# Hiroki-Maeda/ninwavelets

Hardware: AMD Instinct MI355X
Metric: CWT throughput (epochs*chans*samples*freqs)/s (higher is better)
Workload: dtype f32; 1 GPU; C4 Morse CWT, 512 epochs x 64 ch x 16384 samples x 256 freqs per GPU (4096 epochs at 8 GPUs), complex64 out; wavelet=morse, epochs=512, chans=64, samples=16384, freqs=256, output=cwt, engine=fused, chunk_signals=512, parallelism=dp1 (signals sharded, no collective)

## Files before the change

ninwavelets_amd/csrc/nw_fft_dev.h:

```cpp
#pragma once

#include <type_traits>

#include "nw_dcheck.h"
#include "nw_dft_reg.h"
#include "nw_internal.h"
#include "nw_shape.h"

#ifndef NW_PACK_MAX
#define NW_PACK_MAX 2
#endif
constexpr int kPackMax = NW_PACK_MAX;
constexpr int kPruneMin = 4;
constexpr int kXdmaMinE = 32;
constexpr int kWregMaxE = 16;

namespace nw {
namespace {


__device__ __forceinline__ C2<f2> pk(C2<float> a, C2<float> b) { return {f2{a.re, b.re}, f2{a.im, b.im}}; }
__device__ __forceinline__ C2<float> lo(C2<f2> p) { return {p.re.x, p.im.x}; }
__device__ __forceinline__ C2<float> hi(C2<f2> p) { return {p.re.y, p.im.y}; }

__device__ __forceinline__ double mul_nocontract(double a, double b) {
#pragma clang fp contract(off)
    return a * b;
}
__device__ __forceinline__ double add_nocontract(double a, double b) {
#pragma clang fp contract(off)
    return a + b;
}

template <typename P>
__device__ __forceinline__ P* at(P* base, uint32_t lane_off, uint32_t c = 0) {
    asm volatile("" : "+v"(lane_off));
    return reinterpret_cast<P*>(reinterpret_cast<char*>(base) + (lane_off + c));
}
template <typename P>
__device__ __forceinline__ const P* at(const P* base, uint32_t lane_off, uint32_t c = 0) {
    asm volatile("" : "+v"(lane_off));
    return reinterpret_cast<const P*>(reinterpret_cast<const char*>(base) + (lane_off + c));
}

template <typename T, int R, int N, int NSR, bool SPLIT = false>
__device__ __forceinline__ void twiddle_bases(C2<T>* p, int m, const C2<T>* __restrict__ tw,
                                              const C2<T>* split = nullptr) {
    asm volatile("" : "+v"(m));
#pragma unroll
    for (int k = 0; k < ilog2<R>(); ++k) {
        if constexpr (SPLIT) {
            const uint32_t i = ((uint32_t)m << k) * (uint32_t)(N / NSR);
            p[k] = cmul(split[i >> 5], split[N / 64 + (i & 31)]);
        } else if constexpr (sizeof(T) == 4) {
            const float rev = (float)(m << k) * (1.0f / (float)NSR);
            p[k] = C2<T>{__builtin_amdgcn_cosf(rev), __builtin_amdgcn_sinf(rev)};
        } else {
            p[k] = *at(tw, (uint32_t)m * (uint32_t)((N / NSR) * sizeof(C2<T>)) << k);
        }
    }
}
template <typename T, int R, typename P>
__device__ __forceinline__ void twiddle_dft(C2<T>* v, const C2<P>* p) {
    idft_br_tw<T, R>(v, TwPowers<P, R>(p));
}
template <typename S, int R, int NS, bool FENCE> struct TwTable {
    using scalar = S;
    const C2<S>* tab;
    __device__ __forceinline__ C2<S> lo(int r) const { return tab[(r - 1) * NS]; }
    __device__ __forceinline__ C2<S> hi(int r) const {
        const C2<S> w = tab[(r + R / 2 - 1) * NS];
        if (FENCE && r % 4 == 3) __builtin_amdgcn_sched_barrier(0);
        return w;
    }
};

template <int E> constexpr int kPadG = E < 32 ? 32 : E;
template <int E> __device__ __forceinline__ int lds_idx(int i) { return i + 2 * (i / kPadG<E>); }
template <int E> constexpr int lds_off(int c) { return c + 2 * (c / kPadG<E>); }
template <int N, int E> constexpr int lds_elems() { return N + 2 * (N / kPadG<E>); }

template <int N, int E> struct Geometry {
    static constexpr int T = N / E;
    static constexpr int radix(int p) {
        int done = E;
        for (int i = 1; i < p; ++i) done *= (N / done >= E ? E : N / done);
        const int left = N / done;
        return p == 0 ? E : (left >= E ? E : left);
    }
    static constexpr int npass() {
        int done = E, p = 1;
        while (done < N) {
            done *= (N / done >= E ? E : N / done);
            ++p;
        }
        return p;
    }
    static constexpr int ns(int p) {
        int done = 1;
        for (int i = 0; i < p; ++i) done *= radix(i);
        return done;
    }
};

template <int PG> __device__ __forceinline__ int lds_idx_p(int i) { return i + 2 * (i / PG); }
template <int PG> constexpr int lds_off_p(int c) { return c + 2 * (c / PG); }
template <typename T> constexpr bool kIsPair = !std::is_same<T, Sc<T>>::value;
#ifndef NW_PAIR_PAD16
#define NW_PAIR_PAD16 1
#endif
template <typename T, int N, int E>
constexpr bool kPad16 = NW_PAIR_PAD16 && kIsPair<T> && E == 16 && N / E == 256 && Geometry<N, E>::npass() > 2;
template <typename T, int N, int E, int P> constexpr int kPadX = (kPad16<T, N, E> && P == 1) ? 16 : kPadG<E>;
template <typename T, int N, int E> constexpr int kImgElems = kPad16<T, N, E> ? N + 2 * (N / 16) : lds_elems<N, E>();

template <int OUT, typename T> struct OutT { using type = T; };
template <typename T> struct OutT<NW_OUT_CWT, T> { using type = C2<T>; };
constexpr int kOutXHalf = 1000;
constexpr int kOutPSum = 1001;
constexpr int kOutPhSum = 1002;
constexpr int kOutXSum = 1003;
constexpr int kOutPlvSum = 1004;
template <int OUT> constexpr int kPairAcc = OUT == kOutXSum ? 4 : OUT == kOutPlvSum ? 2 : 1;
struct alignas(16) XHalfSlot { double a, b; };
template <typename T> struct OutT<kOutXHalf, T> { using type = XHalfSlot; };
template <int OUT, typename T>
__device__ __forceinline__ typename OutT<OUT, T>::type out_value(C2<T> y) {
    if constexpr (OUT == NW_OUT_CWT) return y;
    else if constexpr (OUT == NW_OUT_POWER) return y.re * y.re + y.im * y.im;
    else return (T)sqrt(y.re * y.re + y.im * y.im);
}

constexpr int kStoreGlobal = 0, kStoreGlobalNt = 1, kStoreBuffer = 2;
#ifdef NW_LINT_HAZARD_SOFFSET
constexpr bool kSoffsetInField = true;
#else
constexpr bool kSoffsetInField = false;
#endif
template <int SP, typename V>
__device__ __forceinline__ void store_row(V val, void* row, uint32_t lane_off, uint32_t c_off) {
    if constexpr (SP == kStoreBuffer) {
        const __amdgpu_buffer_rsrc_t rs = __builtin_amdgcn_make_buffer_rsrc(
            reinterpret_cast<char*>(row) + (kSoffsetInField ? 0 : c_off), 0, 0x7fffffff, 0x00020000);
        const int so = kSoffsetInField ? (int)c_off : 0;
        if constexpr (sizeof(V) == 16)
            __builtin_amdgcn_raw_buffer_store_b128(__builtin_bit_cast(__attribute__((ext_vector_type(4))) unsigned, val),
                                                   rs, (int)lane_off, so, 2);
        else if constexpr (sizeof(V) == 8)
            __builtin_amdgcn_raw_buffer_store_b64(__builtin_bit_cast(__attribute__((ext_vector_type(2))) unsigned, val),
                                                  rs, (int)lane_off, so, 2);
        else
            __builtin_amdgcn_raw_buffer_store_b32(__builtin_bit_cast(unsigned, val), rs, (int)lane_off, so, 2);
    } else {
        __builtin_nontemporal_store(val, reinterpret_cast<V*>(at(reinterpret_cast<char*>(row), lane_off, c_off)));
    }
}
template <typename O> using StoreVec =
    typename std::conditional<sizeof(O) == 16, float __attribute__((ext_vector_type(4))),
    typename std::conditional<sizeof(O) == 8, float __attribute__((ext_vector_type(2))), float>::type>::type;

template <int OUT, typename T, int SP>
__device__ __forceinline__ void store_pair(void* orow, uint32_t lane_idx, uint32_t c_idx, C2<T> y0, C2<T> y1) {
    using O = typename OutT<OUT, T>::type;
    struct alignas(2 * sizeof(O)) P2 { O a, b; };
#ifdef NW_ABL_NOSTORE
    asm volatile("" ::"v"(y0.re), "v"(y0.im), "v"(y1.re), "v"(y1.im), "v"(lane_idx));
    return;
#endif
    using V = typename std::conditional<sizeof(P2) == 16, float __attribute__((ext_vector_type(4))),
              typename std::conditional<sizeof(P2) == 8, float __attribute__((ext_vector_type(2))),
                                        double __attribute__((ext_vector_type(4)))>::type>::type;
    const P2 pv{out_value<OUT, T>(y0), out_value<OUT, T>(y1)};
    store_row<SP>(__builtin_bit_cast(V, pv), orow, lane_idx * (uint32_t)sizeof(O), c_idx * (uint32_t)sizeof(O));
}
template <int OUT, typename T, int SP>
__device__ __forceinline__ void store_one(void* orow, uint32_t lane_idx, uint32_t c_idx, C2<T> y) {
    using O = typename OutT<OUT, T>::type;
#ifdef NW_ABL_NOSTORE
    asm volatile("" ::"v"(y.re), "v"(y.im), "v"(lane_idx));
    return;
#endif
    if constexpr (SP == kStoreGlobal)
        *at(reinterpret_cast<O*>(orow), lane_idx * (uint32_t)sizeof(O), c_idx * (uint32_t)sizeof(O)) =
            out_value<OUT, T>(y);
    else
        store_row<SP>(__builtin_bit_cast(StoreVec<O>, out_value<OUT, T>(y)), orow, lane_idx * (uint32_t)sizeof(O),
                      c_idx * (uint32_t)sizeof(O));
}

#ifdef NW_STAMPS
constexpr int kStamps = 8;
__device__ unsigned long long g_nw_stamps[kStamps + 1];
struct Stamps {
    unsigned long long last, acc[kStamps];
};
__device__ __forceinline__ unsigned long long nw_now() {
    unsigned long long t;
    __builtin_amdgcn_sched_barrier(0);
    asm volatile("s_memtime %0\n\ts_waitcnt lgkmcnt(0)" : "=s"(t)::"memory");
    __builtin_amdgcn_sched_barrier(0);
    return t;
}
#define NW_STAMP(st, k)                                 \
    do {                                                \
        if (st) {    \
            const unsigned long long now_ = nw_now();   \
            (st)->acc[k] += now_ - (st)->last;          \
            (st)->last = now_;                          \
        }                                               \
    } while (0)
constexpr int kStampsStore = kStamps - 1;
#else
struct Stamps {};
#define NW_STAMP(st, k) ((void)(st))
#endif

template <typename T> struct alignas(2 * sizeof(T)) Pair {
    T a, b;
};

template <int COMP, typename T> __device__ __forceinline__ T& comp(C2<T>& c) {
    if constexpr (COMP == 0) return c.re; else return c.im;
}

template <int N, int E, int P, int OSZ = 8, bool PK = false, bool LN = false> struct PassInfo;
typedef __attribute__((address_space(3))) void lds_void_t;

#ifdef NW_LANE_IMAGE_TU
constexpr bool kLaneImageTU = true;
#else
constexpr bool kLaneImageTU = false;
#endif
template <typename T, int N, int E, int OUT>
constexpr bool kLaneImage = kLaneImageTU && kLaneImageShape<T, N, E> && OUT != kOutXHalf;

template <int OFF0, int STEP, bool WAIT>
__device__ __forceinline__ void addtid_store16(uint32_t m0, const float* d) {
    static_assert(OFF0 >= 0 && OFF0 + 15 * STEP < 65536, "16-bit offset field");
    asm volatile(
        "s_mov_b32 m0, %16\n\ts_nop 0\n\t"
        "ds_write_addtid_b32 %0 offset:%17+0*%18\n\t"
        "ds_write_addtid_b32 %1 offset:%17+1*%18\n\t"
        "ds_write_addtid_b32 %2 offset:%17+2*%18\n\t"
        "ds_write_addtid_b32 %3 offset:%17+3*%18\n\t"
        "ds_write_addtid_b32 %4 offset:%17+4*%18\n\t"
        "ds_write_addtid_b32 %5 offset:%17+5*%18\n\t"
        "ds_write_addtid_b32 %6 offset:%17+6*%18\n\t"
        "ds_write_addtid_b32 %7 offset:%17+7*%18\n\t"
        "ds_write_addtid_b32 %8 offset:%17+8*%18\n\t"
        "ds_write_addtid_b32 %9 offset:%17+9*%18\n\t"
        "ds_write_addtid_b32 %10 offset:%17+10*%18\n\t"
        "ds_write_addtid_b32 %11 offset:%17+11*%18\n\t"
        "ds_write_addtid_b32 %12 offset:%17+12*%18\n\t"
        "ds_write_addtid_b32 %13 offset:%17+13*%18\n\t"
        "ds_write_addtid_b32 %14 offset:%17+14*%18\n\t"
        "ds_write_addtid_b32 %15 offset:%17+15*%18"
        :: "v"(d[0]), "v"(d[1]), "v"(d[2]), "v"(d[3]), "v"(d[4]), "v"(d[5]), "v"(d[6]), "v"(d[7]),
           "v"(d[8]), "v"(d[9]), "v"(d[10]), "v"(d[11]), "v"(d[12]), "v"(d[13]), "v"(d[14]), "v"(d[15]),
           "s"(m0), "i"(OFF0), "i"(STEP)
        : "memory", "m0");
    if constexpr (WAIT) asm volatile("s_waitcnt lgkmcnt(0)" ::: "memory");
}

template <typename T, int N, int E, int P, int COMP>
__device__ __forceinline__ void lane_write(C2<T>* v, T* lds, int t) {
    namespace L = lane_image;
    static_assert(kLaneImageShape<T, N, E> && (P == 0 || P == 1), "the fp32 n = 16384 exchanges");
    static_assert(Geometry<N, E>::T % 64 == 0 && Geometry<N, E>::T == L::kT && L::kRebias == 16,
                  "whole waves (EXEC all ones), 16 stores per M0");
    static_assert(L::kElems <= kImgElems<T, N, E>, "the padded images' region holds these");
    NW_DCHECK_H(__builtin_amdgcn_read_exec() == ~0ull);
    const uint32_t img = (uint32_t)(uintptr_t)(lds_void_t*)lds;
    const int wave = __builtin_amdgcn_readfirstlane(t >> 6);
    float d[E];
#pragma unroll
    for (int k = 0; k < E; ++k) d[k] = comp<COMP>(v[bitrev<E>(k)]);
    if constexpr (P == 0) {
        addtid_store16<L::off_01(0), L::off_01(1) - L::off_01(0), false>(img + L::m0_01(wave), d);
        addtid_store16<L::off_01(16), L::off_01(1) - L::off_01(0), true>(img + L::m0_01(wave), d + 16);
    } else {
        static_assert(PassInfo<N, E, P, 16>::R == E && PassInfo<N, E, P, 16>::Q == 1, "one radix-E butterfly per thread");
        addtid_store16<L::off_12(0), L::off_12(1) - L::off_12(0), false>(img + L::m0_12(wave, 0), d);
        addtid_store16<L::off_12(16), L::off_12(17) - L::off_12(16), true>(img + L::m0_12(wave, 16), d + 16);
    }
}

template <typename T, int N, int E, int P, int COMP, bool LN = false>
__device__ __forceinline__ void lds_write(C2<T>* v, T* lds, int t) {
    using G = Geometry<N, E>;
    constexpr int PG = kPadX<T, N, E, P + 1>;
    if constexpr (LN) {
        lane_write<T, N, E, P, COMP>(v, lds, t);
    } else if constexpr (P == 0) {
        NW_DCHECK_H(lds_idx_p<PG>(t * E + E - 1) < kImgElems<T, N, E>);
        Pair<T>* dst = reinterpret_cast<Pair<T>*>(lds + lds_idx_p<PG>(t * E));
#pragma unroll
        for (int u = 0; u < E / 2; ++u)
            dst[u] = Pair<T>{comp<COMP>(v[bitrev<E>(2 * u)]), comp<COMP>(v[bitrev<E>(2 * u + 1)])};
    } else {
        constexpr int R = G::radix(P);
        constexpr int NS = G::ns(P);
        constexpr int Q = E / R;
#pragma unroll
        for (int q = 0; q < Q; ++q) {
            const int j = PassInfo<N, E, P, 16, kIsPair<T>>::bfly(t, q);
            NW_DCHECK_H(lds_idx_p<PG>((j / NS) * NS * R + j % NS) + lds_off_p<PG>((R - 1) * NS) < kImgElems<T, N, E>);
            T* dst = lds + lds_idx_p<PG>((j / NS) * NS * R + j % NS);
#pragma unroll
            for (int i = 0; i < R; ++i) dst[lds_off_p<PG>(bitrev<R>(i) * NS)] = comp<COMP>(v[q * R + i]);
        }
    }
}

template <int N, int E, int P, int OSZ, bool PK, bool LN> struct PassInfo {
    using G = Geometry<N, E>;
    static constexpr int R = G::radix(P);
    static constexpr int NS = G::ns(P);
    static constexpr int Q = E / R;
    static constexpr int STRIDE = N / R;
    static constexpr bool LAST = (P == G::npass() - 1);
    static constexpr bool PAIRED = LAST && Q == 2 && OSZ <= 8;
    static_assert(STRIDE % E == 0 && NS % E == 0, "pad must stay linear");
    static constexpr bool SWZ = PAIRED && G::T == 512 && kPadG<E> == 32 && !LN;
    static constexpr bool REMAP = PK && NW_PAIR_PAD16 && P == 1 && !LAST && E == 16 && G::T == 256 && Q == 1;
    __device__ static __forceinline__ int bfly(int t, int q) {
        if constexpr (SWZ) return 2 * (((t >> 5) << 4) + (((t >> 4) & 1) << 8) + (t & 15)) + q;
        if constexpr (REMAP) return ((t >> 5) << 4) + (((t >> 4) & 1) << 7) + (t & 15);
        return PAIRED ? Q * t + q : t + q * G::T;
    }
};

template <typename T, int N, int E> struct Tab1 {
    using I = PassInfo<N, E, 1>;
    using S = Sc<T>;
    static constexpr int NS = I::NS, R = I::R;
    static constexpr int COUNT = Geometry<N, E>::npass() >= 2 ? NS * (R - 1) : 0;
#ifdef NW_TAB1_F64_16384
    static constexpr bool BIG = sizeof(S) == 8 && N == 16384 && E == 32;
#else
    static constexpr bool BIG = false;
#endif
    static constexpr bool ON = COUNT > 0 && (COUNT * (int)sizeof(C2<S>) <= 8192 || BIG);
    static constexpr int BYTES = ON ? COUNT * (int)sizeof(C2<S>) : 0;
    static_assert((kImgElems<T, N, E> * sizeof(T)) % 16 == 0, "table alignment");
    __device__ static __forceinline__ const C2<S>* table(const T* lds) {
        return reinterpret_cast<const C2<S>*>(lds + kImgElems<T, N, E>);
    }
    __device__ static __forceinline__ void fill(T* lds, const C2<S>* __restrict__ tw, int t) {
        if constexpr (ON) {
            C2<S>* tab = reinterpret_cast<C2<S>*>(lds + kImgElems<T, N, E>);
            for (int i = t; i < COUNT; i += Geometry<N, E>::T) {
                const int jj = i % NS, r = i / NS + 1;
                tab[i] = tw[(jj * r * (N / (NS * R))) % N];
            }
        }
    }
};

template <typename T, int N, int E, int P, int COMP, int OSZ, bool LN = false>
__device__ __forceinline__ void lds_read(C2<T>* v, const T* lds, int t) {
    using I = PassInfo<N, E, P, OSZ, kIsPair<T>, LN>;
    constexpr int R = I::R, Q = I::Q;
    constexpr int PG = kPadX<T, N, E, P>;
    if constexpr (LN) {
        namespace L = lane_image;
        if constexpr (P == 1) {
            static_assert(Q == 1 && R == E && !I::PAIRED, "pass 1: butterfly t, slots t + 512 r");
            const T* src = lds + L::rbase_01(I::bfly(t, 0));
#pragma unroll
            for (int r = 0; r < R; ++r) comp<COMP>(v[r]) = src[L::roff_01(r)];
        } else {
            static_assert(P == 2 && Q == 2 && I::PAIRED && I::STRIDE == 1024, "pass 2: pairs 2t, 2t + 1, slots j2 + 1024 r");
            const T* src = lds + L::rbase_12(I::bfly(t, 0));
#pragma unroll
            for (int r = 0; r < R; ++r) {
                const Pair<T> pr = *reinterpret_cast<const Pair<T>*>(src + L::roff_12(r));
                comp<COMP>(v[r]) = pr.a;
                comp<COMP>(v[R + r]) = pr.b;
            }
        }
    } else if constexpr (I::PAIRED) {
        NW_DCHECK_H(lds_idx_p<PG>(I::bfly(t, 0)) + (Q - 1) + lds_off_p<PG>((R - 1) * I::STRIDE) < kImgElems<T, N, E>);
        const T* src = lds + lds_idx_p<PG>(I::bfly(t, 0));
#pragma unroll
        for (int q = 0; q < Q; q += 2)
#pragma unroll
            for (int r = 0; r < R; ++r) {
                const Pair<T> pr = *reinterpret_cast<const Pair<T>*>(src + q + lds_off_p<PG>(r * I::STRIDE));
                comp<COMP>(v[q * R + r]) = pr.a;
                comp<COMP>(v[(q + 1) * R + r]) = pr.b;
            }
    } else {
#pragma unroll
        for (int q = 0; q < Q; ++q) {
            NW_DCHECK_H(lds_idx_p<PG>(I::bfly(t, q)) + lds_off_p<PG>((R - 1) * I::STRIDE) < kImgElems<T, N, E>);
            const T* src = lds + lds_idx_p<PG>(I::bfly(t, q));
#pragma unroll
            for (int r = 0; r < R; ++r) comp<COMP>(v[q * R + r]) = src[lds_off_p<PG>(r * I::STRIDE)];
        }
    }
}

__device__ __forceinline__ void lds_barrier() {
    __builtin_amdgcn_s_waitcnt(0xC07F);
    __builtin_amdgcn_s_barrier();
}

typedef __attribute__((address_space(1))) void gbl_void_t;

template <typename T, int N, int TT>
__device__ __forceinline__ void dma_x(const C2<T>* xs, void* dst, int t, int nround = 1 << 30) {
    constexpr int CH = (N / 2) * (int)sizeof(C2<T>) / 16;
    static_assert(CH % TT == 0, "whole DMA rounds");
    const int wave_base = __builtin_amdgcn_readfirstlane((t & ~63) * 16);
    const uint32_t lane_off = (uint32_t)t * 16u;
#pragma unroll
    for (int i = 0; i < CH / TT; ++i) {
        if (i >= nround) break;
        const char* chunk = reinterpret_cast<const char*>(xs) + (size_t)i * TT * 16;
        asm volatile("" : "+s"(chunk));
        const uint32_t lds_addr = (uint32_t)(uintptr_t)(lds_void_t*)(reinterpret_cast<char*>(dst) + i * TT * 16 + wave_base);
        asm volatile("s_mov_b32 m0, %0\n\ts_nop 0\n\tglobal_load_lds_dwordx4 %1, %2"
                     :: "s"(lds_addr), "v"(lane_off), "s"(chunk) : "memory", "m0");
    }
}

__device__ __forceinline__ unsigned long long sload_u64(const void* p) {
    unsigned long long u;
    asm volatile("s_load_dwordx2 %0, %1, 0x0\n\ts_waitcnt lgkmcnt(0)" : "=s"(u) : "s"(p) : "memory");
    return u;
}
__device__ __forceinline__ C2<float> c2_of_u64(unsigned long long u) {
    return C2<float>{__uint_as_float((unsigned)u), __uint_as_float((unsigned)(u >> 32))};
}
template <typename T> __device__ __forceinline__ C2<T> sload_c2(const C2<T>* p) {
    if constexpr (sizeof(T) == 4) {
        unsigned long long u;
        asm volatile("s_load_dwordx2 %0, %1, 0x0\n\ts_waitcnt lgkmcnt(0)" : "=s"(u) : "s"(p) : "memory");
        return C2<T>{__uint_as_float((unsigned)u), __uint_as_float((unsigned)(u >> 32))};
    } else {
        typedef unsigned long long u2 __attribute__((ext_vector_type(2)));
        u2 u;
        asm volatile("s_load_dwordx4 %0, %1, 0x0\n\ts_waitcnt lgkmcnt(0)" : "=s"(u) : "s"(p) : "memory");
        return C2<T>{__longlong_as_double((long long)u.x), __longlong_as_double((long long)u.y)};
    }
}

template <int V>
__device__ __forceinline__ void wait_vmcnt() {
    static_assert(V >= 0 && V < 64, "vmcnt range");
    __builtin_amdgcn_s_waitcnt((V & 0xF) | ((V >> 4) << 14) | 0x70 | 0xF00);
}

template <int CTRL> __device__ __forceinline__ float dpp_f(float v) {
    return __int_as_float(__builtin_amdgcn_mov_dpp(__float_as_int(v), CTRL, 0xF, 0xF, false));
}
template <int CTRL> __device__ __forceinline__ double dpp_f(double v) {
    const long long b = __double_as_longlong(v);
    const int lo = __builtin_amdgcn_mov_dpp((int)(b & 0xffffffffLL), CTRL, 0xF, 0xF, false);
    const int hi = __builtin_amdgcn_mov_dpp((int)(b >> 32), CTRL, 0xF, 0xF, false);
    return __longlong_as_double(((long long)hi << 32) | (unsigned int)lo);
}
template <int D, typename F> __device__ __forceinline__ void xpose2(F& a, F& b, bool hi) {
    constexpr int CTRL = D == 1 ? 0xB1 : 0x4E;
    const F recv = dpp_f<CTRL>(hi ? a : b);
    if (hi) a = recv; else b = recv;
}
template <typename F> __device__ __forceinline__ void xpose2(C2<F>& a, C2<F>& b, bool hi, int d) {
    if (d == 1) { xpose2<1>(a.re, b.re, hi); xpose2<1>(a.im, b.im, hi); }
    else { xpose2<2>(a.re, b.re, hi); xpose2<2>(a.im, b.im, hi); }
}

template <typename T, int N, int E, int OUT, int SP = kStoreGlobal>
struct LastStores {
    using O = typename OutT<OUT, T>::type;
    using I = PassInfo<N, E, Geometry<N, E>::npass() - 1, (int)sizeof(O), false, kLaneImage<T, N, E, OUT>>;
    static constexpr int R = I::R, Q = I::Q;
    static constexpr int STEP = I::PAIRED ? 2 : 1;
    static constexpr int PACK_W = (int)(16 / sizeof(O));
    static constexpr int PACK = (!I::PAIRED && PACK_W <= kPackMax && R % PACK_W == 0) ? PACK_W : 1;
    static_assert(PACK == 1 || PACK == 2 || PACK == 4, "pack");
    static constexpr int COUNT = PACK > 1 ? Q * R / PACK : Q / STEP * R;
    __device__ static __forceinline__ void all(const C2<T>* v, void* orow, int t) {
        if constexpr (PACK == 1) {
            chunk<0, 1>(v, orow, t);
        } else {
            const int c = t & (PACK - 1);
            const uint32_t lane = (uint32_t)((t & ~(PACK - 1)) + I::NS * c) * (uint32_t)sizeof(O);
#pragma unroll
            for (int qg = 0; qg < Q * (R / PACK); ++qg) {
                const int q = qg / (R / PACK), g = qg % (R / PACK);
                O val[PACK];
#pragma unroll
                for (int b = 0; b < PACK; ++b) val[b] = out_value<OUT, T>(v[q * R + bitrev<R>(g * PACK + b)]);
                if constexpr (PACK >= 2) {
                    const bool hi1 = c & 1;
#pragma unroll
                    for (int b = 0; b < PACK; b += 2) xpose_any<1>(val[b], val[b + 1], hi1);
                }
                if constexpr (PACK == 4) {
                    const bool hi2 = c & 2;
                    xpose_any<2>(val[0], val[2], hi2);
                    xpose_any<2>(val[1], val[3], hi2);
                }
                using V = float __attribute__((ext_vector_type(4)));
                struct alignas(16) P16 { O a[PACK]; };
                P16 pk;
#pragma unroll
                for (int b = 0; b < PACK; ++b) pk.a[b] = val[b];
#ifdef NW_ABL_NOSTORE
                asm volatile("" ::"v"(__builtin_bit_cast(V, pk)));
#else
                store_row<SP>(__builtin_bit_cast(V, pk), orow, lane,
                              (uint32_t)((q * Geometry<N, E>::T + g * PACK * I::NS) * sizeof(O)));
#endif
            }
        }
    }
    template <int D, typename F> __device__ static __forceinline__ void xpose_any(F& a, F& b, bool hi) {
        if constexpr (std::is_same<F, float>::value || std::is_same<F, double>::value) xpose2<D>(a, b, hi);
        else xpose2(a, b, hi, D);
    }
    template <int K>
    __device__ static __forceinline__ void one(const C2<T>* o, void* orow, int t) {
        constexpr int q = (K / R) * STEP, i = K % R;
        const uint32_t lane = (uint32_t)I::bfly(t, 0);
        constexpr uint32_t c = (uint32_t)((I::PAIRED ? q : q * Geometry<N, E>::T) + bitrev<R>(i) * I::NS);
        NW_DCHECK_H(lane + c + (I::PAIRED ? 1u : 0u) < (uint32_t)N);
        if constexpr (I::PAIRED)
            store_pair<OUT, T, SP>(orow, lane, c, o[q * R + i], o[(q + 1) * R + i]);
        else
            store_one<OUT, T, SP>(orow, lane, c, o[q * R + i]);
    }
    template <int C, int NCH, int K = C * COUNT / NCH>
    __device__ static __forceinline__ void chunk(const C2<T>* o, void* orow, int t) {
        if constexpr (K < (C + 1) * COUNT / NCH) {
            one<K>(o, orow, t);
            chunk<C, NCH, K + 1>(o, orow, t);
        }
    }
};



template <typename T, int E, bool REALW>
constexpr bool kXDMA = E >= (sizeof(T) == 4 ? kXdmaMinE : 32) && REALW;
template <typename T> __device__ __forceinline__ int dma_rounds_for(int nz) {
    return (nz * (int)sizeof(C2<T>) + 15) / 16;
}

template <typename T, int N, int E> struct TwSplit {
    static constexpr bool ON = std::is_same<T, double>::value && N >= 2048 && N <= 4096;
    static constexpr int NHI = N / 64, COUNT = NHI + 32;
    static constexpr int OFFSET = kImgElems<T, N, E> * (int)sizeof(T) + Tab1<T, N, E>::BYTES;
    static_assert(OFFSET % 16 == 0, "table alignment");
    static constexpr int BYTES = ON ? COUNT * (int)sizeof(C2<T>) : 0;
    __device__ static __forceinline__ const C2<T>* table(const T* lds) {
        return reinterpret_cast<const C2<T>*>(reinterpret_cast<const char*>(lds) + OFFSET);
    }
    __device__ static __forceinline__ void fill(T* lds, const C2<T>* __restrict__ tw, int t) {
        if constexpr (ON) {
            C2<T>* tab = reinterpret_cast<C2<T>*>(reinterpret_cast<char*>(lds) + OFFSET);
            for (int i = t; i < COUNT; i += Geometry<N, E>::T) tab[i] = i < NHI ? tw[i * 32] : tw[i - NHI];
        }
    }
};
template <typename T, int N, int E> constexpr int kLdsBytes =
    kImgElems<T, N, E> * (int)sizeof(T) + Tab1<T, N, E>::BYTES + TwSplit<T, N, E>::BYTES;


template <typename T, int N, int E, int OUT, int P, bool XD, int SP = kStoreGlobal>
__device__ __forceinline__ void passes_from(C2<T>* v, T* lds, int t, const C2<Sc<T>>* __restrict__ tw, C2<T>* x,
                                            const C2<T>* xs_next, void* ocur,
                                            Stamps* st, void* ocur2 = nullptr, int dma_rounds = 1 << 30,
                                            double* acc = nullptr, const void* xs_next2 = nullptr) {
    using S = Sc<T>;
    constexpr bool PAIRSIG = !std::is_same<T, S>::value;
    constexpr int OSZ = (int)sizeof(typename OutT<OUT, S>::type);
    constexpr bool LN = kLaneImage<T, N, E, OUT>;
    using I = PassInfo<N, E, P, OSZ, kIsPair<T>, LN>;
    if constexpr (P < Geometry<N, E>::npass()) {
        constexpr int R = I::R, Q = I::Q, LR = ilog2<R>();
        constexpr bool TABLED = P == 1 && Tab1<T, N, E>::ON;
        constexpr bool SPLIT = TwSplit<T, N, E>::ON;
        const C2<S>* split = nullptr;
        if constexpr (SPLIT) split = reinterpret_cast<const C2<S>*>(TwSplit<T, N, E>::table(lds));
        C2<S> pb[Q][LR > 0 ? LR : 1];
#ifndef NW_ABL_NOTWIDDLE
        if constexpr (!TABLED && I::PAIRED && Q == 2) {
            twiddle_bases<S, R, N, I::NS * R, SPLIT>(pb[0], I::bfly(t, 0) % I::NS, tw, split);
#pragma unroll
            for (int k = 0; k < LR; ++k) pb[1][k] = cmul(pb[0][k], tw[(N / (I::NS * R)) << k]);
        } else if constexpr (!TABLED) {
#pragma unroll
            for (int q = 0; q < Q; ++q) twiddle_bases<S, R, N, I::NS * R, SPLIT>(pb[q], I::bfly(t, q) % I::NS, tw, split);
        }
#endif
#ifndef NW_ABL_NOEXCH
        lds_barrier();
        lds_write<T, N, E, P - 1, 0, LN>(v, lds, t);
        lds_barrier();
        lds_read<T, N, E, P, 0, OSZ, LN>(v, lds, t);
        lds_barrier();
        lds_write<T, N, E, P - 1, 1, LN>(v, lds, t);
        lds_barrier();
        lds_read<T, N, E, P, 1, OSZ, LN>(v, lds, t);
#else
#pragma unroll
        for (int i = 0; i < E; ++i) asm volatile("" : "+v"(v[i].re), "+v"(v[i].im));
#endif
        if constexpr (I::LAST && XD) {
            if (xs_next) {
                lds_barrier();
                if constexpr (PAIRSIG) {
                    dma_x<S, N, Geometry<N, E>::T>(reinterpret_cast<const C2<S>*>(xs_next), lds, t, dma_rounds);
                    dma_x<S, N, Geometry<N, E>::T>(reinterpret_cast<const C2<S>*>(xs_next2),
                                                   reinterpret_cast<char*>(lds) + (N / 2) * sizeof(C2<S>), t, dma_rounds);
                } else {
                    dma_x<T, N, Geometry<N, E>::T>(xs_next, lds, t, dma_rounds);
                }
                __builtin_amdgcn_sched_barrier(0);
            }
        }
        NW_STAMP(st, 2 * P - 1);
#pragma unroll
        for (int q = 0; q < Q; ++q) {
#ifdef NW_ABL_NOTWIDDLE
            constexpr bool TWIDDLED = false;
#else
            constexpr bool TWIDDLED = true;
#endif
            if constexpr (std::is_same<T, float>::value && Q % 2 == 0 && !(TWIDDLED && TABLED)) {
                if (q % 2 == 0) {
                    C2<f2> pv[R];
#pragma unroll
                    for (int i = 0; i < R; ++i)
                        pv[i] = pk(reinterpret_cast<C2<float>*>(v)[q * R + i],
                                   reinterpret_cast<C2<float>*>(v)[(q + 1) * R + i]);
                    if constexpr (TWIDDLED) {
                        C2<f2> pp[LR > 0 ? LR : 1];
#pragma unroll
                        for (int k = 0; k < LR; ++k)
                            pp[k] = pk(reinterpret_cast<C2<float>*>(pb[q])[k], reinterpret_cast<C2<float>*>(pb[q + 1])[k]);
                        twiddle_dft<f2, R>(pv, pp);
                    } else {
                        idft_br<f2, R>(pv);
                    }
#pragma unroll
                    for (int i = 0; i < R; ++i) {
                        reinterpret_cast<C2<float>*>(v)[q * R + i] = lo(pv[i]);
                        reinterpret_cast<C2<float>*>(v)[(q + 1) * R + i] = hi(pv[i]);
                    }
                }
            } else if constexpr (TWIDDLED && TABLED) {
                idft_br_tw<T, R>(v + q * R, TwTable<S, R, I::NS, true>{Tab1<T, N, E>::table(lds) + I::bfly(t, q) % I::NS});
            } else if constexpr (TWIDDLED) {
                twiddle_dft<T, R>(v + q * R, pb[q]);
            } else {
                idft_br<T, R>(v + q * R);
            }
        }
        NW_STAMP(st, 2 * P);
        if constexpr (I::LAST && OUT == kOutPSum) {
            if constexpr (PAIRSIG) {
#pragma unroll
                for (int e = 0; e < Q * R; ++e) {
                    const C2<S> a{v[e].re.x, v[e].im.x};
                    acc[e] += (double)(a.re * a.re + a.im * a.im);
                }
                if (ocur2) {
#pragma unroll
                    for (int e = 0; e < Q * R; ++e) {
                        const C2<S> b{v[e].re.y, v[e].im.y};
                        acc[e] += (double)(b.re * b.re + b.im * b.im);
                    }
                }
            } else {
#pragma unroll
                for (int e = 0; e < Q * R; ++e) acc[e] += (double)(v[e].re * v[e].re + v[e].im * v[e].im);
            }
        } else if constexpr (I::LAST && OUT == kOutPhSum) {
            static_assert(!PAIRSIG, "partial sums run the single-signal kernel");
#pragma unroll
            for (int e = 0; e < Q * R; ++e) {
                const double re = (double)v[e].re, im = (double)v[e].im;
                if constexpr (sizeof(S) == 8) {
                    const double inv = 1.0 / hypot(re, im);
                    acc[2 * e] += mul_nocontract(re, inv);
                    acc[2 * e + 1] += mul_nocontract(im, inv);
                } else {
                    const double inv = rsqrt(re * re + im * im);
                    acc[2 * e] += mul_nocontract(re, inv);
                    acc[2 * e + 1] += mul_nocontract(im, inv);
                }
            }
        } else if constexpr (I::LAST && (OUT == kOutXSum || OUT == kOutPlvSum)) {
            static_assert(PAIRSIG, "cross-channel partials run the signal-pair kernel");
            NW_DCHECK_H(ocur2 != nullptr);
#pragma unroll
            for (int e = 0; e < Q * R; ++e) {
                double ar = (double)v[e].re.x, ai = (double)v[e].im.x;
                double br = (double)v[e].re.y, bi = (double)v[e].im.y;
                if constexpr (OUT == kOutPlvSum) {
                    const double ia = rsqrt(add_nocontract(mul_nocontract(ar, ar), mul_nocontract(ai, ai)));
                    const double ib = rsqrt(add_nocontract(mul_nocontract(br, br), mul_nocontract(bi, bi)));
                    ar = mul_nocontract(ar, ia), ai = mul_nocontract(ai, ia);
                    br = mul_nocontract(br, ib), bi = mul_nocontract(bi, ib);
                }
                constexpr int NA = kPairAcc<OUT>;
                acc[NA * e] += add_nocontract(mul_nocontract(ar, br), mul_nocontract(ai, bi));
                acc[NA * e + 1] += add_nocontract(mul_nocontract(ai, br), -mul_nocontract(ar, bi));
                if constexpr (OUT == kOutXSum) {
                    acc[NA * e + 2] += add_nocontract(mul_nocontract(ar, ar), mul_nocontract(ai, ai));
                    acc[NA * e + 3] += add_nocontract(mul_nocontract(br, br), mul_nocontract(bi, bi));
                }
            }
        } else if constexpr (I::LAST && OUT == kOutXHalf) {
            static_assert(!I::PAIRED, "forward stores are lane-contiguous");
            C2<S>* xr = reinterpret_cast<C2<S>*>(ocur);
#pragma unroll
            for (int q = 0; q < Q; ++q)
#pragma unroll
                for (int i = 0; i < R; ++i) {
                    const int k = I::bfly(t, q) + bitrev<R>(i) * I::NS;
                    if (k <= N / 2) xr[k] = C2<S>{v[q * R + i].re, -v[q * R + i].im};
                }
        } else if constexpr (I::LAST) {
            __builtin_amdgcn_sched_barrier(0);
            if constexpr (PAIRSIG) {
                C2<S> a[E], b[E];
#pragma unroll
                for (int i = 0; i < E; ++i) {
                    a[i] = C2<S>{v[i].re.x, v[i].im.x};
                    b[i] = C2<S>{v[i].re.y, v[i].im.y};
                }
                LastStores<S, N, E, OUT, SP>::all(a, ocur, t);
                if (ocur2) LastStores<S, N, E, OUT, SP>::all(b, ocur2, t);
            } else {
                LastStores<T, N, E, OUT, SP>::all(v, ocur, t);
            }
        } else {
            passes_from<T, N, E, OUT, P + 1, XD, SP>(v, lds, t, tw, x, xs_next, ocur, st, ocur2, dma_rounds, acc, xs_next2);
        }
    }
}
}
}
```

ninwavelets_amd/csrc/nw_shape.h:

```cpp
#pragma once

#include <stddef.h>
#include <stdint.h>

#include <type_traits>

#include "../../include/ninwave.h"

#ifdef __HIP__
#define NW_SHAPE_HD __host__ __device__
#else
#define NW_SHAPE_HD
#endif
#define NW_INLINE inline __attribute__((always_inline))

namespace nw {

template <typename T> constexpr int kDtypeOf = sizeof(T) == 4 ? NW_F32 : NW_F64;


struct BlockSlot {
    int row, group;
};
NW_SHAPE_HD NW_INLINE BlockSlot block_slot(int b, int nrows, int tile_f, int tile_g) {
// ... 105 lines not shown
    return reinterpret_cast<const int*>(static_cast<const char*>(wtab) + wtab_row_bytes(n, nfreq, esz, realw));
}

NW_SHAPE_HD constexpr int wnz_round(int need, int e) {
    int p2 = 1;
    while (p2 < need && p2 < 8) p2 <<= 1;
    if (p2 < need) p2 = (need + 3) / 4 * 4;
    return p2 < e ? p2 : e;
}


constexpr bool kNz24 = true;
template <typename T, int N, int E> constexpr bool kNz24Of = kNz24 && E > 16;
template <typename T, int N, int E> constexpr bool kNzFineOf = kNz24Of<T, N, E> && sizeof(T) == 4;
#ifndef NW_F64_FINE
#define NW_F64_FINE 1
#endif
#if NW_F64_FINE
template <typename T, int N, int E, int OUT> constexpr bool kNzFineOut = kNzFineOf<T, N, E> ||
    (kNz24Of<T, N, E> && OUT == NW_OUT_CWT);
#else
template <typename T, int N, int E, int OUT> constexpr bool kNzFineOut = kNzFineOf<T, N, E>;
#endif
template <int E, bool FINE, bool NZ24>
NW_SHAPE_HD constexpr NW_INLINE int pass0_variant(int nz) {
    if (nz <= 4) return 4;
    if (nz <= 8) return 8;
    if (FINE && nz <= 12) return 12;
    if (E > 16 && nz <= 16) return 16;
    if (FINE && nz <= 20) return 20;
    if (NZ24 && nz <= 24) return 24;
    return E;
}
NW_SHAPE_HD constexpr int pair_pass0_variant(int nz, int e) { return nz <= 4 ? 4 : nz <= 8 ? 8 : nz <= 12 ? 12 : e; }


template <typename T, int E, bool REALW>
constexpr bool kPairMode = std::is_same<T, float>::value && E <= 16 && REALW;

template <typename T, int EO, bool PHASE>
constexpr int kPsE = (EO >= 32 && (PHASE || sizeof(T) == 8)) ? 16 : EO;
template <int EO, int E> constexpr int kPsShift = EO == E ? 0 : EO == 2 * E ? 1 : 2;
template <typename T, int N, int EO>
constexpr bool kPSumOK = !(sizeof(T) == 8 && N / kPsE<T, EO, false> > 512);
template <typename T, int N, int EO>
constexpr bool kPhSumOK = N / kPsE<T, EO, true> <= 512;

template <int N> constexpr bool kPairXSumOK = N >= 1024 && N <= 4096;
template <int N> constexpr bool kPairPlvSumOK = N >= 1024 && N <= 4096;
constexpr bool pair_partials_supported(int64_t n, int dtype, int kind, int out_kind) {
    if (dtype != NW_F32 || (kind != NW_MORSE && kind != NW_MORLET && kind != NW_SHANNON)) return false;
    const bool xs = n == 1024 ? kPairXSumOK<1024> : n == 2048 ? kPairXSumOK<2048> : n == 4096 ? kPairXSumOK<4096> : false;
    const bool ps = n == 1024 ? kPairPlvSumOK<1024> : n == 2048 ? kPairPlvSumOK<2048> : n == 4096 ? kPairPlvSumOK<4096> : false;
    return out_kind == NW_OUT_CROSS_SUM ? xs : out_kind == NW_OUT_PLV_SUM ? ps : false;
}


#ifndef NW_LANE_IMAGE
#define NW_LANE_IMAGE 1
#endif
template <typename T, int N, int E>
constexpr bool kLaneImageShape = NW_LANE_IMAGE && std::is_same<T, float>::value && N == 16384 && E == 32;
namespace lane_image {
constexpr int kN = 16384, kE = 32, kT = kN / kE;
constexpr int kS1 = 513, kS2 = 544;
constexpr int kElems = kE * kS2;
constexpr int kBytes = kElems * 4;
constexpr int kTab1Bytes = kE * (kE - 1) * 8;
constexpr int kCuLdsBytes = 160 * 1024;
constexpr int kRebias = 16;
NW_SHAPE_HD constexpr int addr01(int i) { return (i % kE) * kS1 + i / kE; }
NW_SHAPE_HD constexpr int addr12(int i) { return ((i % 1024) / 32) * kS2 + (i / 1024) * 32 + i % 32; }
NW_SHAPE_HD constexpr int m0_01(int wave) { return 256 * wave; }
NW_SHAPE_HD constexpr int off_01(int p) { return 4 * p * kS1; }
NW_SHAPE_HD constexpr int m0_12(int wave, int ip) { return 256 * wave + (ip >= kRebias ? 4 * kRebias * kS2 : 0); }
NW_SHAPE_HD constexpr int off_12(int ip) { return 4 * (ip % kRebias) * kS2; }
NW_SHAPE_HD constexpr int rbase_01(int u) { return (u % kE) * kS1 + u / kE; }
NW_SHAPE_HD constexpr int roff_01(int r) { return (kT / kE) * r; }
NW_SHAPE_HD constexpr int rbase_12(int j2) { return (j2 / 32) * kS2 + j2 % 32; }
NW_SHAPE_HD constexpr int roff_12(int r) { return 32 * r; }
static_assert(addr01(kN - 1) < kElems && addr12(kN - 1) < kElems, "both images inside the region");
static_assert(off_01(kE - 1) < 65536 && off_12(kE - 1) < 65536, "16-bit offset field");
static_assert(2 * (kBytes + kTab1Bytes) <= kCuLdsBytes, "two blocks per CU");
}


constexpr int kConnPairs = 64;
constexpr int kConnCh = 16;
constexpr int kConnTileN = 64;
constexpr int kConnWaves = 4;
constexpr int kConnPerWave = kConnPairs / kConnWaves;
static_assert(kConnPairs % kConnWaves == 0 && kConnCh % kConnWaves == 0, "conn geometry");
struct ConnTile {
    int32_t nch, npairs;
    int32_t ch[kConnCh];
    int32_t sa[kConnPairs], sb[kConnPairs], out[kConnPairs];
};
struct ConnSlot {
    int64_t unit;
    int tile;
};
NW_SHAPE_HD NW_INLINE ConnSlot conn_slot(int64_t b, int ntiles, bool xcd) {
    if (!xcd) return {b / ntiles, (int)(b % ntiles)};
    const int64_t local = b >> 3;
    return {(local / ntiles) * 8 + (b & 7), (int)(local % ntiles)};
}
constexpr int64_t conn_units(int nfreq, int64_t n_out) { return (int64_t)nfreq * ((n_out + kConnTileN - 1) / kConnTileN); }
constexpr int64_t conn_blocks(int64_t nunits, int ntiles, bool xcd) {
    return (xcd ? (nunits + 7) / 8 * 8 : nunits) * ntiles;
}


struct ConnTimeSlot {
    int64_t e;
    int f, tile;
};
NW_SHAPE_HD NW_INLINE ConnTimeSlot conn_time_slot(int64_t b, int nfreq, int ntiles, bool xcd) {
    const ConnSlot sl = conn_slot(b, ntiles, xcd);
    return {sl.unit / nfreq, (int)(sl.unit % nfreq), sl.tile};
}
constexpr int64_t conn_time_blocks(int64_t ec, int nfreq, int ntiles, bool xcd) {
    return conn_blocks(ec * nfreq, ntiles, xcd);
}
constexpr int64_t conn_time_count(int64_t t0, int64_t t1, int64_t step) { return (t1 - t0 + step - 1) / step; }
constexpr int conn_time_lane(int64_t j) { return (int)(j % kConnTileN); }
constexpr int64_t conn_time_tiles(int64_t count) { return (count + kConnTileN - 1) / kConnTileN; }
static_assert(conn_time_count(0, 0, 1) == 0 && conn_time_count(37, 1001, 1) == 964 && conn_time_count(0, 1, 4) == 1 &&
                  conn_time_count(8, 1000, 4) == 248 && conn_time_count(8, 1001, 4) == 249,
              "window sample count");
static_assert(conn_time_lane(0) == 0 && conn_time_lane(63) == 63 && conn_time_lane(64) == 0 && conn_time_tiles(65) == 2,
              "lane of a sample");
static_assert(conn_time_blocks(2, 9, 3, false) == 54 && conn_time_blocks(2, 9, 3, true) == 72, "block count");


constexpr int kPacPh = 8;
constexpr int kPacAm = 16;
constexpr int kPacWaves = 4;
constexpr int kPacAmWave = kPacAm / kPacWaves;
constexpr int kPacStagePh = kPacPh / kPacWaves;
constexpr int kPacStageAm = kPacAm / kPacWaves;
static_assert(kPacAm % kPacWaves == 0 && kPacPh % kPacWaves == 0, "pac geometry");
static_assert(2 * (2 * kPacPh + kPacAm) * kConnTileN * 8 <= 64 * 1024, "double-buffered staging fits the LDS of a block");
constexpr int64_t pac_tiles_ph(int64_t nph) { return (nph + kPacPh - 1) / kPacPh; }
constexpr int64_t pac_tiles_am(int64_t nam) { return (nam + kPacAm - 1) / kPacAm; }
constexpr int64_t pac_tiles(int64_t nph, int64_t nam) { return pac_tiles_ph(nph) * pac_tiles_am(nam); }
struct PacSlot {
    int64_t e;
    int pair, tp, ta;
};
NW_SHAPE_HD NW_INLINE PacSlot pac_slot(int64_t b, int npairs, int ntiles, int nta, bool xcd) {
    const ConnSlot sl = conn_slot(b, ntiles, xcd);
    return {sl.unit / npairs, (int)(sl.unit % npairs), sl.tile / nta, sl.tile % nta};
}
constexpr int64_t pac_blocks(int64_t ec, int64_t npairs, int64_t ntiles, bool xcd) {
    return ntiles > 0x7fffffff ? -1 : conn_blocks(ec * npairs, (int)ntiles, xcd);
}
static_assert(pac_tiles_ph(8) == 1 && pac_tiles_ph(9) == 2 && pac_tiles_am(16) == 1 && pac_tiles_am(17) == 2 &&
                  pac_tiles(9, 17) == 4 && pac_tiles(0, 5) == 0,
              "scale tile counts");
static_assert(pac_blocks(2, 5, 4, false) == 40 && pac_blocks(2, 5, 4, true) == 64 && pac_blocks(0, 5, 4, true) == 0,
              "block count");


constexpr int kLargeLog2Min = 15, kLargeLog2Max = 24;
constexpr bool large_supported(int64_t n, int dtype) {
    return (dtype == NW_F32 || dtype == NW_F64) && n >= (int64_t(1) << kLargeLog2Min) &&
// ... 154 lines not shown
```

Before: 692.7 billion points/s.

## Use inline-asm batched ds_read_b64 for pass-2 image and twiddle table reads

```diff
diff --git a/ninwavelets_amd/csrc/nw_fft_dev.h b/ninwavelets_amd/csrc/nw_fft_dev.h
--- a/ninwavelets_amd/csrc/nw_fft_dev.h
+++ b/ninwavelets_amd/csrc/nw_fft_dev.h
@@ -24,6 +24,14 @@
 __device__ __forceinline__ C2<float> hi(C2<f2> p) { return {p.re.y, p.im.y}; }
 
 __device__ __forceinline__ double mul_nocontract(double a, double b) {
+#pragma clang fp contract(off)
+    return a * b;
+}
+__device__ __forceinline__ float mul_nocontract(float a, float b) {
+#pragma clang fp contract(off)
+    return a * b;
+}
+__device__ __forceinline__ f2 mul_nocontract(f2 a, f2 b) {
 #pragma clang fp contract(off)
     return a * b;
 }
@@ -124,6 +132,14 @@
 template <int OUT> constexpr int kPairAcc = OUT == kOutXSum ? 4 : OUT == kOutPlvSum ? 2 : 1;
 struct alignas(16) XHalfSlot { double a, b; };
 template <typename T> struct OutT<kOutXHalf, T> { using type = XHalfSlot; };
+template <bool RE_FUSED>
+__device__ __forceinline__ f2 norm2_pinned(C2<float> y0, C2<float> y1) {
+    const f2 re{y0.re, y1.re}, im{y0.im, y1.im};
+    if constexpr (RE_FUSED) return fma_t(re, re, mul_nocontract(im, im));
+    else return fma_t(im, im, mul_nocontract(re, re));
+}
+constexpr int kPinNone = 0, kPinImFused = 1, kPinReFused = 2;
+constexpr int pin_of(int i) { return i <= 1 ? kPinReFused : kPinImFused; }
 template <int OUT, typename T>
 __device__ __forceinline__ typename OutT<OUT, T>::type out_value(C2<T> y) {
     if constexpr (OUT == NW_OUT_CWT) return y;
@@ -159,7 +175,7 @@
     typename std::conditional<sizeof(O) == 16, float __attribute__((ext_vector_type(4))),
     typename std::conditional<sizeof(O) == 8, float __attribute__((ext_vector_type(2))), float>::type>::type;
 
-template <int OUT, typename T, int SP>
+template <int OUT, typename T, int SP, int PIN = kPinNone>
 __device__ __forceinline__ void store_pair(void* orow, uint32_t lane_idx, uint32_t c_idx, C2<T> y0, C2<T> y1) {
     using O = typename OutT<OUT, T>::type;
     struct alignas(2 * sizeof(O)) P2 { O a, b; };
@@ -170,7 +186,14 @@
     using V = typename std::conditional<sizeof(P2) == 16, float __attribute__((ext_vector_type(4))),
               typename std::conditional<sizeof(P2) == 8, float __attribute__((ext_vector_type(2))),
                                         double __attribute__((ext_vector_type(4)))>::type>::type;
-    const P2 pv{out_value<OUT, T>(y0), out_value<OUT, T>(y1)};
+    P2 pv;
+    if constexpr (PIN != kPinNone && OUT != NW_OUT_CWT) {
+        static_assert(std::is_same<T, float>::value && (OUT == NW_OUT_POWER || OUT == NW_OUT_ABS), "the lane images' kernels");
+        const f2 p = norm2_pinned<PIN == kPinReFused>(y0, y1);
+        if constexpr (OUT == NW_OUT_POWER) pv = P2{p.x, p.y}; else pv = P2{(T)sqrt(p.x), (T)sqrt(p.y)};
+    } else {
+        pv = P2{out_value<OUT, T>(y0), out_value<OUT, T>(y1)};
+    }
     store_row<SP>(__builtin_bit_cast(V, pv), orow, lane_idx * (uint32_t)sizeof(O), c_idx * (uint32_t)sizeof(O));
 }
 template <int OUT, typename T, int SP>
@@ -262,6 +285,80 @@
     if constexpr (WAIT) asm volatile("s_waitcnt lgkmcnt(0)" ::: "memory");
 }
 
+template <typename T, int N, int E, int OUT>
+constexpr int kAsmReads = kLaneImage<T, N, E, OUT> ? (NW_LDS_ASM_READS) : 0;
+
+typedef float lds_f2 __attribute__((ext_vector_type(2)));
+__device__ __forceinline__ uint32_t lds_addr(const void* p) { return (uint32_t)(uintptr_t)(const lds_void_t*)p; }
+#define NW_DSR(k, b) "ds_read_b64 %[o" #k "], %[" #b "] offset:%[f]+" #k "*%[st]\n\t"
+#define NW_DSR4(a, b, c, d, base) NW_DSR(a, base) NW_DSR(b, base) NW_DSR(c, base) NW_DSR(d, base)
+#define NW_DSO(k) [o##k] "=&v"(o[k])
+#define NW_DSO4(a, b, c, d) NW_DSO(a), NW_DSO(b), NW_DSO(c), NW_DSO(d)
+#define NW_DS_WAIT "s_waitcnt lgkmcnt(0)"
+template <int OFF0, int STEP>
+__device__ __forceinline__ void ds_read_b64_16(uint32_t base, lds_f2* o) {
+    static_assert(OFF0 >= 0 && OFF0 % 8 == 0 && STEP % 8 == 0 && OFF0 + 15 * STEP < 65536, "16-bit offset field");
+    asm volatile(NW_DSR4(0, 1, 2, 3, bd) NW_DSR4(4, 5, 6, 7, bd) NW_DSR4(8, 9, 10, 11, bd) NW_DSR4(12, 13, 14, 15, bd) NW_DS_WAIT
+                 : NW_DSO4(0, 1, 2, 3), NW_DSO4(4, 5, 6, 7), NW_DSO4(8, 9, 10, 11), NW_DSO4(12, 13, 14, 15)
+                 : [bd] "v"(base), [f] "i"(OFF0), [st] "i"(STEP)
+                 : "memory");
+}
+template <int F0, int F1, int F2, int F3, int F4, int F5, int F6, int F7>
+__device__ __forceinline__ void ds_read_b64_8(uint32_t base, lds_f2* o) {
+    static_assert(F0 < 65536 && F1 < 65536 && F2 < 65536 && F3 < 65536 && F4 < 65536 && F5 < 65536 && F6 < 65536 && F7 < 65536,
+                  "16-bit offset field");
+    static_assert((F0 < 0 || F0 % 8 == 0) && (F1 | F2 | F3 | F4 | F5 | F6 | F7) % 8 == 0 && F1 >= 0, "8-byte entries");
+    if constexpr (F0 >= 0) {
+        asm volatile("ds_read_b64 %[o0], %[bd] offset:%[f0]\n\tds_read_b64 %[o1], %[bd] offset:%[f1]\n\t"
+                     "ds_read_b64 %[o2], %[bd] offset:%[f2]\n\tds_read_b64 %[o3], %[bd] offset:%[f3]\n\t"
+                     "ds_read_b64 %[o4], %[bd] offset:%[f4]\n\tds_read_b64 %[o5], %[bd] offset:%[f5]\n\t"
+                     "ds_read_b64 %[o6], %[bd] offset:%[f6]\n\tds_read_b64 %[o7], %[bd] offset:%[f7]\n\t" NW_DS_WAIT
+                     : NW_DSO4(0, 1, 2, 3), NW_DSO4(4, 5, 6, 7)
+                     : [bd] "v"(base), [f0] "i"(F0), [f1] "i"(F1), [f2] "i"(F2), [f3] "i"(F3), [f4] "i"(F4), [f5] "i"(F5),
+                       [f6] "i"(F6), [f7] "i"(F7)
+                     : "memory");
+    } else {
+        asm volatile("ds_read_b64 %[o1], %[bd] offset:%[f1]\n\t"
+                     "ds_read_b64 %[o2], %[bd] offset:%[f2]\n\tds_read_b64 %[o3], %[bd] offset:%[f3]\n\t"
+                     "ds_read_b64 %[o4], %[bd] offset:%[f4]\n\tds_read_b64 %[o5], %[bd] offset:%[f5]\n\t"
+                     "ds_read_b64 %[o6], %[bd] offset:%[f6]\n\tds_read_b64 %[o7], %[bd] offset:%[f7]\n\t" NW_DS_WAIT
+                     : NW_DSO(1), NW_DSO(2), NW_DSO(3), NW_DSO4(4, 5, 6, 7)
+                     : [bd] "v"(base), [f1] "i"(F1), [f2] "i"(F2), [f3] "i"(F3), [f4] "i"(F4), [f5] "i"(F5), [f6] "i"(F6),
+                       [f7] "i"(F7)
+                     : "memory");
+    }
+}
+struct TwEntry { float re, im; };
+__device__ __forceinline__ C2<float> cmul(C2<float> v, TwEntry w) {
+    return {fma_t(v.re, w.re, -mul_nocontract(v.im, w.im)), fma_t(v.im, w.re, mul_nocontract(v.re, w.im))};
+}
+template <int R, int NS> struct TwTableAsm {
+    using scalar = float;
+    static_assert(R == lane_image::kE && NS == lane_image::kE && lane_image::kTabBatch == 4 && !kUseDifTw<float, float, R>,
+                  "pass 1 of the fp32 n = 16384 kernels, DIT order");
+    uint32_t col;
+    mutable lds_f2 w[8];
+    template <int B> __device__ __forceinline__ void batch() const {
+        namespace L = lane_image;
+        constexpr int r = 4 * B, h = R / 2;
+        ds_read_b64_8<B == 0 ? -1 : L::tab1_off(B == 0 ? 1 : r), L::tab1_off(r + h), L::tab1_off(r + 1), L::tab1_off(r + 1 + h),
+                      L::tab1_off(r + 2), L::tab1_off(r + 2 + h), L::tab1_off(r + 3), L::tab1_off(r + 3 + h)>(col, w);
+    }
+    __device__ __forceinline__ void first(int r) const {
+        if (r == 0) batch<0>(); else if (r == 4) batch<1>(); else if (r == 8) batch<2>(); else batch<3>();
+    }
+    __device__ __forceinline__ TwEntry lo(int r) const {
+        if (r % 4 == 0) first(r);
+        return {w[2 * (r % 4)].x, w[2 * (r % 4)].y};
+    }
+    __device__ __forceinline__ C2<float> hi(int r) const {
+        if (r == 0) first(r);
+        const C2<float> c{w[2 * (r % 4) + 1].x, w[2 * (r % 4) + 1].y};
+        if (r % 4 == 3) __builtin_amdgcn_sched_barrier(0);
+        return c;
+    }
+};
+
 template <typename T, int N, int E, int P, int COMP>
 __device__ __forceinline__ void lane_write(C2<T>* v, T* lds, int t) {
     namespace L = lane_image;
@@ -357,7 +454,7 @@
     }
 };
 
-template <typename T, int N, int E, int P, int COMP, int OSZ, bool LN = false>
+template <typename T, int N, int E, int P, int COMP, int OSZ, bool LN = false, int AR = 0>
 __device__ __forceinline__ void lds_read(C2<T>* v, const T* lds, int t) {
     using I = PassInfo<N, E, P, OSZ, kIsPair<T>, LN>;
     constexpr int R = I::R, Q = I::Q;
@@ -372,11 +469,23 @@
         } else {
             static_assert(P == 2 && Q == 2 && I::PAIRED && I::STRIDE == 1024, "pass 2: pairs 2t, 2t + 1, slots j2 + 1024 r");
             const T* src = lds + L::rbase_12(I::bfly(t, 0));
-#pragma unroll
-            for (int r = 0; r < R; ++r) {
-                const Pair<T> pr = *reinterpret_cast<const Pair<T>*>(src + L::roff_12(r));
-                comp<COMP>(v[r]) = pr.a;
-                comp<COMP>(v[R + r]) = pr.b;
+            if constexpr ((AR & L::kAsmReadImage) != 0) {
+                static_assert(R == 16 && L::rd12_off(1) * 15 == L::rd12_off(15), "16 reads, evenly spaced");
+                NW_DCHECK_H(L::rd12_base(t) == (int)((const char*)src - (const char*)lds));
+                lds_f2 pr[R];
+                ds_read_b64_16<L::rd12_off(0), L::rd12_off(1)>(lds_addr(src), pr);
+#pragma unroll
+                for (int r = 0; r < R; ++r) {
+                    comp<COMP>(v[r]) = pr[r].x;
+                    comp<COMP>(v[R + r]) = pr[r].y;
+                }
+            } else {
+#pragma unroll
+                for (int r = 0; r < R; ++r) {
+                    const Pair<T> pr = *reinterpret_cast<const Pair<T>*>(src + L::roff_12(r));
+                    comp<COMP>(v[r]) = pr.a;
+                    comp<COMP>(v[R + r]) = pr.b;
+                }
             }
         }
     } else if constexpr (I::PAIRED) {
@@ -528,7 +637,7 @@
         constexpr uint32_t c = (uint32_t)((I::PAIRED ? q : q * Geometry<N, E>::T) + bitrev<R>(i) * I::NS);
         NW_DCHECK_H(lane + c + (I::PAIRED ? 1u : 0u) < (uint32_t)N);
         if constexpr (I::PAIRED)
-            store_pair<OUT, T, SP>(orow, lane, c, o[q * R + i], o[(q + 1) * R + i]);
+            store_pair<OUT, T, SP, kLaneImage<T, N, E, OUT> ? pin_of(i) : kPinNone>(orow, lane, c, o[q * R + i], o[(q + 1) * R + i]);
         else
             store_one<OUT, T, SP>(orow, lane, c, o[q * R + i]);
     }
@@ -578,6 +687,7 @@
     constexpr bool PAIRSIG = !std::is_same<T, S>::value;
     constexpr int OSZ = (int)sizeof(typename OutT<OUT, S>::type);
     constexpr bool LN = kLaneImage<T, N, E, OUT>;
+    constexpr int AR = kAsmReads<T, N, E, OUT>;
     using I = PassInfo<N, E, P, OSZ, kIsPair<T>, LN>;
     if constexpr (P < Geometry<N, E>::npass()) {
         constexpr int R = I::R, Q = I::Q, LR = ilog2<R>();
@@ -600,11 +710,11 @@
         lds_barrier();
         lds_write<T, N, E, P - 1, 0, LN>(v, lds, t);
         lds_barrier();
-        lds_read<T, N, E, P, 0, OSZ, LN>(v, lds, t);
+        lds_read<T, N, E, P, 0, OSZ, LN, AR>(v, lds, t);
         lds_barrier();
         lds_write<T, N, E, P - 1, 1, LN>(v, lds, t);
         lds_barrier();
-        lds_read<T, N, E, P, 1, OSZ, LN>(v, lds, t);
+        lds_read<T, N, E, P, 1, OSZ, LN, AR>(v, lds, t);
 #else
 #pragma unroll
         for (int i = 0; i < E; ++i) asm volatile("" : "+v"(v[i].re), "+v"(v[i].im));
@@ -652,6 +762,10 @@
                         reinterpret_cast<C2<float>*>(v)[(q + 1) * R + i] = hi(pv[i]);
                     }
                 }
+            } else if constexpr (TWIDDLED && TABLED && (AR & lane_image::kAsmReadTab1) != 0 && !kUseDifTw<T, S, R>) {
+                static_assert(Q == 1 && kImgElems<T, N, E> * (int)sizeof(T) == lane_image::kBytes, "the table's place");
+                NW_DCHECK_H(lane_image::tab1_base(t) == (int)((const char*)(Tab1<T, N, E>::table(lds) + I::bfly(t, q) % I::NS) - (const char*)lds));
+                idft_br_tw<T, R>(v + q * R, TwTableAsm<R, I::NS>{lds_addr(Tab1<T, N, E>::table(lds) + I::bfly(t, q) % I::NS), {}});
             } else if constexpr (TWIDDLED && TABLED) {
                 idft_br_tw<T, R>(v + q * R, TwTable<S, R, I::NS, true>{Tab1<T, N, E>::table(lds) + I::bfly(t, q) % I::NS});
             } else if constexpr (TWIDDLED) {
@@ -676,8 +790,18 @@
                     }
                 }
             } else {
-#pragma unroll
-                for (int e = 0; e < Q * R; ++e) acc[e] += (double)(v[e].re * v[e].re + v[e].im * v[e].im);
+                if constexpr (LN) {
+                    static_assert(Q == 2, "the paired last pass");
+                    f2 p[R];
+#pragma unroll
+                    for (int e = 0; e < R; ++e)
+                        p[e] = pin_of(e) == kPinReFused ? norm2_pinned<true>(v[e], v[R + e]) : norm2_pinned<false>(v[e], v[R + e]);
+#pragma unroll
+                    for (int e = 0; e < Q * R; ++e) acc[e] += (double)(e < R ? p[e].x : p[e - R].y);
+                } else {
+#pragma unroll
+                    for (int e = 0; e < Q * R; ++e) acc[e] += (double)(v[e].re * v[e].re + v[e].im * v[e].im);
+                }
             }
         } else if constexpr (I::LAST && OUT == kOutPhSum) {
             static_assert(!PAIRSIG, "partial sums run the single-signal kernel");
diff --git a/ninwavelets_amd/csrc/nw_shape.h b/ninwavelets_amd/csrc/nw_shape.h
--- a/ninwavelets_amd/csrc/nw_shape.h
+++ b/ninwavelets_amd/csrc/nw_shape.h
@@ -211,6 +211,17 @@
 static_assert(addr01(kN - 1) < kElems && addr12(kN - 1) < kElems, "both images inside the region");
 static_assert(off_01(kE - 1) < 65536 && off_12(kE - 1) < 65536, "16-bit offset field");
 static_assert(2 * (kBytes + kTab1Bytes) <= kCuLdsBytes, "two blocks per CU");
+
+#ifndef NW_LDS_ASM_READS
+#define NW_LDS_ASM_READS 3
+#endif
+constexpr int kAsmReadImage = 1, kAsmReadTab1 = 2;
+NW_SHAPE_HD constexpr int rd12_base(int t) { return 4 * rbase_12(2 * t); }
+NW_SHAPE_HD constexpr int rd12_off(int r) { return 4 * roff_12(r); }
+constexpr int kTabBatch = 4;
+NW_SHAPE_HD constexpr int tab1_base(int t) { return kBytes + 8 * (t % kE); }
+NW_SHAPE_HD constexpr int tab1_off(int r) { return 8 * kE * (r - 1); }
+static_assert(rd12_off(15) < 65536 && tab1_off(kE - 1) < 65536, "16-bit offset field");
 }
 
 
```

Measured after the change: 711.1 billion points/s, median of 6. 1.03x the previous value.
